# JuliaRobotics/KernelDensityEstimate.jl

Hardware: AMD Instinct MI355X
Metric: gibbs_product_samples_per_sec (higher is better)
Workload: dtype f64

## Files before the change

include/kdehip.h:

```cpp
#ifndef KDEHIP_H
#define KDEHIP_H

#include <stdint.h>

#ifdef __cplusplus
extern "C" {
#endif

#define KDEHIP_VERSION 600

enum {
  KDEHIP_OK = 0,
  KDEHIP_ERR_ARG = -1,
  KDEHIP_ERR_DIM_MISMATCH = -2,
  KDEHIP_ERR_RAND_SHORT = -3,
  KDEHIP_ERR_NO_DEVICE = -4,
  KDEHIP_ERR_HIP = -5,
  KDEHIP_ERR_ALLOC = -6,
  KDEHIP_ERR_UNSUPPORTED = -7
};

#define KDEHIP_MAX_DIMS 8
#define KDEHIP_MAX_DENS 16

// ... 19 lines not shown

int kdehip_gibbs1_trace(int Ndens, const kdehip_density *trees, int64_t Np, int Niter, double *pts,
                        int64_t *ind, const double *randU, int64_t nU, const double *randN, int64_t nN,
                        int addEntropy, int ndims, const uint8_t *partialDimMask, int device,
                        int32_t *labels);

int kdehip_gibbs1_multi(int Ndens, const kdehip_density *trees, int64_t Np, int Niter, double *pts,
                        int64_t *ind, const double *randU, int64_t nU, const double *randN, int64_t nN,
                        int addEntropy, int ndims, const uint8_t *partialDimMask, int device, int ngpus,
                        int32_t *labels);

#define KDEHIP_MANIFOLD_EUCLIDEAN 0
#define KDEHIP_MANIFOLD_CIRCULAR 1
int kdehip_gibbs1_manifold(int Ndens, const kdehip_density *trees, int64_t Np, int Niter, double *pts, int64_t *ind,
                           const double *randU, int64_t nU, const double *randN, int64_t nN, int addEntropy, int ndims,
                           const uint8_t *partialDimMask, const uint8_t *manifold , int device,
                           int32_t *labels );

int kdehip_prod_philox(int Ndens, const kdehip_density *trees, int64_t Np, int Niter, double *pts, int64_t *ind,
                       uint64_t seed, int addEntropy, int ndims, const uint8_t *partialDimMask, int precision,
                       int device, int ngpus, int32_t *labels);

typedef struct kdehip_product kdehip_product;

typedef struct kdehip_product_info_t {
  int32_t ndens, ndims, nlevels;
  int32_t precision;
  int64_t nodes_per_sweep;
  int64_t bytes_per_eval;
  int64_t packed_bytes;
  int32_t fast_math_path;
  int32_t device;
} kdehip_product_info_t;

int kdehip_product_create(kdehip_product **out, int Ndens, const kdehip_density *trees, int ndims,
                          const uint8_t *partialDimMask, int precision, int device);
void kdehip_product_destroy(kdehip_product *plan);
int kdehip_product_info(const kdehip_product *plan, kdehip_product_info_t *info);
int64_t kdehip_product_randu_per_sample(const kdehip_product *plan, int Niter);
int64_t kdehip_product_randn_per_sample(const kdehip_product *plan);

int kdehip_product_sample_streams(kdehip_product *plan, int64_t Np, int Niter,
                                  const double *d_randU, int64_t nU, const double *d_randN,
                                  int64_t nN, int addEntropy, double *d_points, int64_t *d_indices,
                                  int32_t *d_labels, void *stream);
int kdehip_product_sample_philox(kdehip_product *plan, int64_t Np, int Niter, uint64_t seed,
                                 int64_t sample_offset, int addEntropy, double *d_points,
                                 int64_t *d_indices, int32_t *d_labels, void *stream);
int kdehip_product_sample_philox_host(kdehip_product *plan, int64_t Np, int Niter, uint64_t seed,
                                      int64_t sample_offset, int addEntropy, double *points,
                                      int64_t *indices, int32_t *labels);
int64_t kdehip_product_fallback_count(kdehip_product *plan);
int kdehip_product_screen_stats(kdehip_product *plan, int32_t *levels, int64_t *steps, int64_t *repeats);
int kdehip_product_set_variant(kdehip_product *plan, int variant);
int kdehip_product_launch_geometry(const kdehip_product *plan, int64_t Np, int32_t *waves_per_workgroup,
                                   int32_t *waves_per_chain);
const char *kdehip_product_kernel_name(const kdehip_product *plan, int64_t Np);

typedef struct kdehip_product_multi kdehip_product_multi;
int kdehip_product_multi_create(kdehip_product_multi **out, int Ndens, const kdehip_density *trees, int ndims,
                                const uint8_t *partialDimMask, int precision, int first_device, int ngpus);
void kdehip_product_multi_destroy(kdehip_product_multi *mp);
int kdehip_product_multi_ngpus(const kdehip_product_multi *mp);
kdehip_product *kdehip_product_multi_plan(kdehip_product_multi *mp, int g);
int kdehip_product_multi_sample_philox(kdehip_product_multi *mp, int64_t Np, int Niter, uint64_t seed,
                                       int64_t sample_offset, int addEntropy, double *const *d_points,
                                       int64_t *const *d_indices, void *const *streams);
int kdehip_product_multi_transfers_per_product(const kdehip_product_multi *mp);

typedef struct kdehip_device_density kdehip_device_density;
int kdehip_density_upload(kdehip_device_density **out, const kdehip_density *host, int device);
void kdehip_density_free(kdehip_device_density *d);
int64_t kdehip_density_npts(const kdehip_device_density *d);
int kdehip_density_ndim(const kdehip_device_density *d);
int kdehip_prod_philox_device(int Ndens, kdehip_device_density *const *trees, int64_t Np, int Niter, uint64_t seed,
                              int64_t sample_offset, int addEntropy, const uint8_t *partialDimMask, int precision,
                              double *d_points, int64_t *d_indices, int32_t *d_labels, void *stream);

int kdehip_prod_philox_resident(int Ndens, kdehip_device_density *const *trees, int64_t Np, int Niter, uint64_t seed,
                                int addEntropy, const uint8_t *partialDimMask, int precision, double *pts, int64_t *ind);

int kdehip_density_from_device_points(kdehip_device_density **out, const double *d_points, int64_t D, int64_t N,
                                      int device, void *stream, double *bw_out, int32_t *nevals);
int kdehip_density_from_device_points_manifold(kdehip_device_density **out, const double *d_points, int64_t D, int64_t N,
                                               int device, void *stream, double *bw_out, int32_t *nevals,
                                               const uint8_t *manifold );
int kdehip_mul_device(kdehip_device_density **out, int Ndens, kdehip_device_density *const *trees, uint64_t seed,
                      int addEntropy, double *bw_out, int32_t *nevals);
typedef struct kdehip_mul_item {
  int32_t Ndens;
  int32_t addEntropy;
  kdehip_device_density *const *trees;
  uint64_t seed;
} kdehip_mul_item;
int kdehip_mul_device_batch(int nprod, const kdehip_mul_item *items, kdehip_device_density **out, double *bw_out,
                            int32_t *nevals);
int kdehip_density_download(const kdehip_device_density *d, double *centers, double *ranges, double *weights,
                            int64_t *left_child, int64_t *right_child, int64_t *lowest_leaf, int64_t *highest_leaf,
                            int64_t *permutation, double *means, double *bandwidth, double *bandwidthMin,
                            double *bandwidthMax, double *bw_out);

typedef struct kdehip_batch_item {
  int32_t Ndens;
  int32_t Niter;
  kdehip_device_density *const *trees;
  int64_t Np;
// ... 135 lines not shown
```

kerneldensityestimate.jl_amd/_lib.py:

```python
from __future__ import annotations

import ctypes as C
import os

_HERE = os.path.dirname(os.path.abspath(__file__))
LIB_PATH = os.environ.get("KDEHIP_LIB", os.path.join(_HERE, "libkdehip.so"))

f64p = C.POINTER(C.c_double)
i64p = C.POINTER(C.c_int64)
i32p = C.POINTER(C.c_int32)
u8p = C.POINTER(C.c_uint8)

KDEHIP_OK = 0
ERR_ARG, ERR_DIM_MISMATCH, ERR_RAND_SHORT, ERR_NO_DEVICE, ERR_HIP, ERR_ALLOC, ERR_UNSUPPORTED = -1, -2, -3, -4, -5, -6, -7
MAX_DIMS, MAX_DENS = 8, 16


class CDensity(C.Structure):
    _fields_ = [
        ("npts", C.c_int64), ("ndim", C.c_int64),
        ("means", f64p), ("bandwidth", f64p), ("weights", f64p),
        ("left_child", i64p), ("right_child", i64p), ("permutation", i64p),
    ]

# ... 25 lines not shown

class CSummaryItem(C.Structure):
    _fields_ = [("density", C.c_void_p), ("extend", C.c_double), ("Ngrid", C.c_int64), ("d_range", C.c_void_p),
                ("d_mean", C.c_void_p), ("d_cov", C.c_void_p), ("d_argmax", C.c_void_p), ("d_values", C.c_void_p)]


class CProductInfo(C.Structure):
    _fields_ = [
        ("ndens", C.c_int32), ("ndims", C.c_int32), ("nlevels", C.c_int32), ("precision", C.c_int32),
        ("nodes_per_sweep", C.c_int64), ("bytes_per_eval", C.c_int64), ("packed_bytes", C.c_int64),
        ("fast_math_path", C.c_int32), ("device", C.c_int32),
    ]


SIGNATURES = {
    "kdehip_version": (C.c_int, []),
    "kdehip_last_error": (C.c_char_p, []),
    "kdehip_device_count": (C.c_int, []),
    "kdehip_clear_cache": (None, []),
    "kdehip_gibbs1": (C.c_int, [C.c_int, C.POINTER(CDensity), C.c_int64, C.c_int, f64p, i64p, f64p, C.c_int64,
                                f64p, C.c_int64, C.c_int, C.c_int, u8p, C.c_int]),
    "kdehip_gibbs1_trace": (C.c_int, [C.c_int, C.POINTER(CDensity), C.c_int64, C.c_int, f64p, i64p, f64p, C.c_int64,
                                      f64p, C.c_int64, C.c_int, C.c_int, u8p, C.c_int, i32p]),
    "kdehip_gibbs1_multi": (C.c_int, [C.c_int, C.POINTER(CDensity), C.c_int64, C.c_int, f64p, i64p, f64p, C.c_int64,
                                      f64p, C.c_int64, C.c_int, C.c_int, u8p, C.c_int, C.c_int, i32p]),
    "kdehip_gibbs1_manifold": (C.c_int, [C.c_int, C.POINTER(CDensity), C.c_int64, C.c_int, f64p, i64p, f64p, C.c_int64,
                                         f64p, C.c_int64, C.c_int, C.c_int, u8p, u8p, C.c_int, i32p]),
    "kdehip_prod_philox": (C.c_int, [C.c_int, C.POINTER(CDensity), C.c_int64, C.c_int, f64p, i64p, C.c_uint64, C.c_int,
                                     C.c_int, u8p, C.c_int, C.c_int, C.c_int, i32p]),
    "kdehip_product_multi_create": (C.c_int, [C.POINTER(C.c_void_p), C.c_int, C.POINTER(CDensity), C.c_int, u8p,
                                              C.c_int, C.c_int, C.c_int]),
    "kdehip_product_multi_destroy": (None, [C.c_void_p]),
    "kdehip_product_multi_ngpus": (C.c_int, [C.c_void_p]),
    "kdehip_product_multi_plan": (C.c_void_p, [C.c_void_p, C.c_int]),
    "kdehip_product_multi_sample_philox": (C.c_int, [C.c_void_p, C.c_int64, C.c_int, C.c_uint64, C.c_int64, C.c_int,
                                                     C.POINTER(C.c_void_p), C.POINTER(C.c_void_p),
                                                     C.POINTER(C.c_void_p)]),
    "kdehip_product_multi_transfers_per_product": (C.c_int, [C.c_void_p]),
    "kdehip_product_create": (C.c_int, [C.POINTER(C.c_void_p), C.c_int, C.POINTER(CDensity), C.c_int, u8p,
                                        C.c_int, C.c_int]),
    "kdehip_product_destroy": (None, [C.c_void_p]),
    "kdehip_product_info": (C.c_int, [C.c_void_p, C.POINTER(CProductInfo)]),
    "kdehip_product_randu_per_sample": (C.c_int64, [C.c_void_p, C.c_int]),
    "kdehip_product_randn_per_sample": (C.c_int64, [C.c_void_p]),
    "kdehip_product_fallback_count": (C.c_int64, [C.c_void_p]),
    "kdehip_product_sample_streams": (C.c_int, [C.c_void_p, C.c_int64, C.c_int, C.c_void_p, C.c_int64,
                                                C.c_void_p, C.c_int64, C.c_int, C.c_void_p, C.c_void_p,
                                                C.c_void_p, C.c_void_p]),
    "kdehip_product_sample_philox": (C.c_int, [C.c_void_p, C.c_int64, C.c_int, C.c_uint64, C.c_int64, C.c_int,
                                               C.c_void_p, C.c_void_p, C.c_void_p, C.c_void_p]),
    "kdehip_product_sample_philox_host": (C.c_int, [C.c_void_p, C.c_int64, C.c_int, C.c_uint64, C.c_int64,
                                                    C.c_int, f64p, i64p, i32p]),
    "kdehip_product_screen_stats": (C.c_int, [C.c_void_p, i32p, i64p, i64p]),
    "kdehip_product_set_variant": (C.c_int, [C.c_void_p, C.c_int]),
    "kdehip_product_launch_geometry": (C.c_int, [C.c_void_p, C.c_int64, i32p, i32p]),
    "kdehip_product_kernel_name": (C.c_char_p, [C.c_void_p, C.c_int64]),
    "kdehip_density_upload": (C.c_int, [C.POINTER(C.c_void_p), C.POINTER(CDensity), C.c_int]),
    "kdehip_density_free": (None, [C.c_void_p]),
    "kdehip_density_npts": (C.c_int64, [C.c_void_p]),
    "kdehip_density_ndim": (C.c_int, [C.c_void_p]),
    "kdehip_prod_philox_device": (C.c_int, [C.c_int, C.POINTER(C.c_void_p), C.c_int64, C.c_int, C.c_uint64, C.c_int64,
                                            C.c_int, u8p, C.c_int, C.c_void_p, C.c_void_p, C.c_void_p, C.c_void_p]),
    "kdehip_prod_philox_resident": (C.c_int, [C.c_int, C.POINTER(C.c_void_p), C.c_int64, C.c_int, C.c_uint64, C.c_int, u8p,
                                              C.c_int, f64p, i64p]),
    "kdehip_philox_fill_uniform": (None, [C.c_uint64, C.c_int64, C.c_int64, C.c_int64, f64p]),
    "kdehip_philox_fill_normal": (None, [C.c_uint64, C.c_int64, C.c_int64, C.c_int64, f64p]),
    "kdehip_evaluate": (C.c_int, [C.POINTER(CDensity), f64p, C.c_int64, C.c_int, f64p, C.c_int]),
    "kdehip_eval_avg_logl": (C.c_int, [C.POINTER(CDensity), C.POINTER(CDensity), C.c_int, f64p, C.c_int]),
    "kdehip_eval_avg_logl_device_batch": (C.c_int, [C.c_int, C.POINTER(CLoglItem), C.c_void_p, C.c_void_p]),
    "kdehip_eval_avg_logl_device": (C.c_int, [C.c_void_p, C.c_void_p, C.c_int, f64p]),
    "kdehip_evaluate_device": (C.c_int, [C.c_void_p, C.c_void_p, C.c_int64, C.c_int, C.c_void_p, C.c_void_p]),
    "kdehip_evaluate_device_at": (C.c_int, [C.c_void_p, C.c_void_p, C.c_void_p, C.c_void_p]),
    "kdehip_evaluate_manifold": (C.c_int, [C.POINTER(CDensity), f64p, C.c_int64, C.c_int, f64p, C.c_int, u8p]),
    "kdehip_evaluate_device_manifold": (C.c_int, [C.c_void_p, C.c_void_p, C.c_int64, C.c_int, C.c_void_p, C.c_void_p, u8p]),
    "kdehip_evaluate_device_at_manifold": (C.c_int, [C.c_void_p, C.c_void_p, C.c_void_p, C.c_void_p, u8p]),
    "kdehip_eval_avg_logl_manifold": (C.c_int, [C.POINTER(CDensity), C.POINTER(CDensity), C.c_int, f64p, C.c_int, u8p]),
    "kdehip_eval_avg_logl_device_manifold": (C.c_int, [C.c_void_p, C.c_void_p, C.c_int, f64p, u8p]),
    "kdehip_eval_avg_logl_device_batch_manifold": (C.c_int, [C.c_int, C.POINTER(CLoglManifoldItem), C.c_void_p, C.c_void_p]),
    "kdehip_auto_bandwidth_manifold": (C.c_int, [C.c_int64, C.c_int64, f64p, f64p, i32p, C.c_int, u8p]),
    "kdehip_make_density_auto_manifold": (C.c_int, [C.c_int64, C.c_int64, f64p, f64p, i32p, C.c_int, f64p, f64p, f64p, i64p,
                                                    i64p, i64p, i64p, i64p, f64p, f64p, f64p, f64p, u8p]),
    "kdehip_density_from_device_points_manifold": (C.c_int, [C.POINTER(C.c_void_p), C.c_void_p, C.c_int64, C.c_int64,
                                                             C.c_int, C.c_void_p, f64p, i32p, u8p]),
    "kdehip_density_marginal_device": (C.c_int, [C.POINTER(C.c_void_p), C.c_void_p, C.c_int, i32p]),
    "kdehip_summary_device_batch": (C.c_int, [C.c_int, C.POINTER(CSummaryItem), C.c_void_p]),
    "kdehip_density_summary": (C.c_int, [C.c_void_p, f64p, C.c_int64, f64p, f64p, f64p, f64p, f64p]),
    "kdehip_kde_max": (C.c_int, [C.POINTER(CDensity), C.c_int64, f64p, f64p, C.c_int]),
    "kdehip_inters_intg_appx_is": (C.c_int, [C.POINTER(CDensity), C.POINTER(CDensity), C.c_int64, f64p, C.c_int]),
    "kdehip_inters_intg_appx_is_device": (C.c_int, [C.c_void_p, C.c_void_p, C.c_int64, f64p]),
    "kdehip_auto_bandwidth": (C.c_int, [C.c_int64, C.c_int64, f64p, f64p, i32p, C.c_int]),
    "kdehip_make_density_device_supported": (C.c_int, [C.c_int64, C.c_int64]),
    "kdehip_make_densities_device": (C.c_int, [C.c_int, C.c_int64, i64p] + [C.POINTER(C.c_void_p)] * 2 + [C.c_int64] +
                                     [C.POINTER(C.c_void_p)] * 13 + [C.c_int]),
    "kdehip_density_set_bandwidth": (C.c_int, [C.c_int64, C.c_int64, f64p, C.c_int64, f64p, i64p, i64p, f64p, f64p, f64p, f64p]),
    "kdehip_profile_sampler": (None, [C.c_int]),
    "kdehip_profile_phase_read": (C.c_int, [C.c_int, f64p, i64p]),
    "kdehip_selftest_fp32": (C.c_int, [C.c_int, C.c_uint32, C.c_uint64, C.c_int, f64p, C.POINTER(C.c_uint32),
                                      C.POINTER(C.c_uint32)]),
    "kdehip_profile_sampler_read": (C.c_int, [C.c_int, C.c_void_p, f64p, i64p]),
    "kdehip_product_multi_timing": (C.c_int, [C.c_void_p, f64p, f64p]),
    "kdehip_density_from_device_points": (C.c_int, [C.POINTER(C.c_void_p), C.c_void_p, C.c_int64, C.c_int64, C.c_int,
                                                    C.c_void_p, f64p, i32p]),
    "kdehip_mul_device": (C.c_int, [C.POINTER(C.c_void_p), C.c_int, C.POINTER(C.c_void_p), C.c_uint64, C.c_int, f64p, i32p]),
    "kdehip_mul_device_batch": (C.c_int, [C.c_int, C.POINTER(CMulItem), C.POINTER(C.c_void_p), f64p, i32p]),
    "kdehip_density_download": (C.c_int, [C.c_void_p, f64p, f64p, f64p, i64p, i64p, i64p, i64p, i64p, f64p, f64p, f64p,
                                          f64p, f64p]),
# ... 64 lines not shown
```

kerneldensityestimate.jl_amd/csrc/gibbs_lean.hip:

```cpp
#define KDEHIP_EXP256 1
#ifndef KDEHIP_PRELOAD_MAXB
#define KDEHIP_PRELOAD_MAXB 8
#endif
#include "gibbs_device.hpp"
#include "screen_device.hpp"

namespace kdehip {

template <int I> using IC = std::integral_constant<int, I>;
template <int N, int I = 0, typename F>
__device__ __forceinline__ void static_for(F &&f) {
  if constexpr (I < N) {
    f(IC<I>{});
    static_for<N, I + 1>(f);
  }
}

#if defined(KDEHIP_LEAN_HI) || (defined(KDEHIP_LEAN_DEV_M) && KDEHIP_LEAN_DEV_M > 4)
constexpr int kLeanMinDens = 8, kLeanMaxDens = 8;
#else
constexpr int kLeanMinDens = 2, kLeanMaxDens = 4;
#endif
constexpr int kLeanMaxNormals = 128;

__device__ __forceinline__ int scalar_copy(int x) {
  int y;
  asm("s_mov_b32 %0, %1" : "=s"(y) : "s"(x));
  return y;
}

template <int D>
struct LeanTile {
  int n;
  int flags;
  int lds_off;
  int stage_bytes;
  int chunk_rows;
  int seg;
  int hdr_lo, hdr_hi;
  int B, F, last_lane;
  int uniform_bw;
  __device__ __forceinline__ int64_t hdr_off() const {
    return (static_cast<int64_t>(hdr_hi) << 32) | static_cast<uint32_t>(hdr_lo);
  }
  __device__ __forceinline__ void load(const kdehip_v8i &d) {
    n = scalar_copy(d[0]);
    flags = scalar_copy(d[1]);
    lds_off = scalar_copy(d[2]);
    stage_bytes = scalar_copy(d[3]);
    chunk_rows = scalar_copy(d[4]);
    seg = scalar_copy(d[5]);
    hdr_lo = scalar_copy(d[6]);
    hdr_hi = scalar_copy(d[7]);
    B = (n + 63) >> 6;
    last_lane = flags & 0xFF;
    uniform_bw = flags >> 8;
    F = uniform_bw ? D + 1 : 2 * D + 1;
  }
};

template <typename P, typename T, bool OK> constexpr bool kCanPreloadImpl = OK && kIsLdsPtr<P> && sizeof(T) == 8;

template <typename T, int D, int M, int WAVES, bool BATCH = false, bool SCHUNK = false>
__global__ __launch_bounds__(WAVES * 64) void gibbs_lean_kernel(PlanDev plan_, RunArgs a_) {
  const LaunchView<BATCH> view(plan_, a_);
  const PlanDev &plan = view.plan;
  const auto &a = view.a;
  constexpr bool kPrefetchRows = (WAVES <= 12) || sizeof(T) == 4 || D <= 4;
  using RowPtr = std::conditional_t<(WAVES == 16 && sizeof(T) == 8), LdsPtrSplit<T>, LdsPtr<T>>;
  constexpr int kCopyWaves = WAVES > 4 ? 4 : WAVES;
  constexpr bool kKeptRows = (WAVES <= 8);
  constexpr bool kScreen = sizeof(T) == 8 && !BATCH;
  constexpr bool kPreloadBuild = kKeptRows && kPrefetchRows;
  constexpr int kNormOff = 2048;
  constexpr int kUnifOff = kNormOff + WAVES * kLeanMaxNormals * 8;
  constexpr int kPoolOff = kUnifOff + WAVES * 1024;
  constexpr bool kCoop = kScreen && SCHUNK && WAVES == 8;
  constexpr int kXchgOff = kPoolOff + kLdsPoolBytes;
  constexpr int kXchgSlotDoubles = 32 + 4 * 64;
  constexpr int kXchgBytes = kCoop ? 64 + WAVES * kXchgSlotDoubles * 8 : 0;
  static_assert(kPoolOff + kLdsPoolBytes + kXchgBytes <= 160 * 1024, "LDS budget of one CU exceeded");
  __shared__ __attribute__((aligned(1024))) unsigned char smem[kPoolOff + kLdsPoolBytes + kXchgBytes];

  double *sExpTab = reinterpret_cast<double *>(smem);
  if (threadIdx.x < 256) sExpTab[threadIdx.x] = kExp2Tab256[threadIdx.x];
  if constexpr (kCoop) {
    if (threadIdx.x < 16) reinterpret_cast<int *>(smem + kXchgOff)[threadIdx.x] = 0;
  }

  const int lane = threadIdx.x & 63;
  const int wave = __builtin_amdgcn_readfirstlane(static_cast<int>(threadIdx.x >> 6));
  KDEHIP_PRIO_CHAIN();
  const int chain = wave;
  int64_t s = static_cast<int64_t>(view.block) * WAVES + chain;
  const bool live = s < a.Np;
  if (!live) s = a.Np - 1;
  const uint64_t gs = static_cast<uint64_t>(a.sample_offset + s);
  const void *fb = live ? static_cast<const void *>(plan.levels) : nullptr;

  const int L = plan.L;
  const T *__restrict__ data = static_cast<const T *>(plan.data);
  const LevelTable levels{(const __attribute__((address_space(4))) kdehip_v16i *)(plan.levels)};
  const StepTable steps{(const __attribute__((address_space(4))) kdehip_v8i *)(plan.levels + 2 * plan.M * (plan.L + 1))};
  unsigned char *pool = smem + kPoolOff;
  const int dl = lane < D ? lane : D - 1;
  const int vlev = a.variant % 1000;

  double *sNorm = reinterpret_cast<double *>(smem + kNormOff) + chain * kLeanMaxNormals;
  const int R = D * (L + 1);
  if (a.rng_philox) {
    for (int b = lane; 2 * b < R; b += 64) {
      double n0, n1;
// ... 636 lines not shown
      const int nsteps = npass * M;
      for (int p = 0; p < npass; ++p)
        static_for<M>([&](auto jc) {
          constexpr int j = decltype(jc)::value;
          constexpr int jn = (j + 1 == M) ? 0 : j + 1;
          const LeanTile<D> ds = tile(j);
          const LeanTile<D> dn = tile(jn);
          T mean = x, cov = T(0);
          if (p != 0) product(jc, mean, cov);
          const double u = next_uniform();
          const T *hdr = data + ds.hdr_off();
          const int pos = draw(ds, hdr, mean, cov, [&](const auto &ev) {
            using Ev = std::decay_t<decltype(ev)>;
            const int RS = TileAddr<T>::stride(ds.F), rc = ds.chunk_rows;
            LaneAcc<T> acc;
            SegSums<T> seg;
            const int cps = seg_chunks(ds.seg);
            const bool use_seg = cps != 0;
            int cin = 0;
            KDEHIP_PRIO_ROWS();
            for (int r0 = 0; r0 < ds.B; r0 += rc, ++gchunk) {
              staging_barrier();
              if (r0 + rc < ds.B) stage_chunk(ds, r0 + rc, (gchunk + 1) & 1);
              else if (t + 1 < nsteps) stage_chunk(dn, 0, (gchunk + 1) & 1);
              const int nrows = (ds.B - r0 < rc) ? (ds.B - r0) : rc;
              const auto crows = (RowPtr)(pool + (gchunk & 1) * (kLdsPoolBytes / 2));
              lane_rows_all<T, RowPtr, Ev, kPrefetchRows>(crows, nrows, RS, lane, ev, acc);
              if (use_seg && ++cin == cps) { seg.note(acc.total()); cin = 0; }
            }
            KDEHIP_PRIO_CHAIN();
            const T S = acc.total();
            if (use_seg)
              return __builtin_amdgcn_readfirstlane(
                  select_or_raise_seg<T, const T *>(S, seg, cps * rc, hdr + kTileHeader, ds, lane, ev, u, fb));
            return __builtin_amdgcn_readfirstlane(select_or_raise<T, const T *>(S, hdr + kTileHeader, ds, lane, ev, u, fb));
          });
          adopt(jc, ds, hdr, pos);
          ++t;
        });
    } else {
      for (int p = 0; p < npass; ++p)
        static_for<M>([&](auto jc) {
          const LeanTile<D> ds = tile(decltype(jc)::value);
          step(jc, ds, data + ds.hdr_off(), p == 0, x);
        });
    }

    if (tabulated) {
      TabDesc td[M];
      static_for<M>([&](auto jc) { td[decltype(jc)::value] = tabs[decltype(jc)::value * (L + 1) + l]; });
      uint32_t word = 0;
      static_for<M>([&](auto jc) { word |= static_cast<uint32_t>(psel[decltype(jc)::value]) << td[decltype(jc)::value].shift; });
      word = __builtin_amdgcn_readfirstlane(word);
      for (int p = 1; p <= a.Niter; ++p)
        static_for<M>([&](auto jc) {
          constexpr int j = decltype(jc)::value;
          const TabDesc &tj = td[j];
          const uint32_t cfg = (word & ((1u << tj.shift) - 1u)) | ((word >> (tj.shift + tj.bits)) << tj.shift);
          const T *row = tables + tj.off + static_cast<int64_t>(cfg) * (tj.n + 1);
          const int n = tj.n;
          const T incl = row[lane < n ? lane : n];
          const double u = next_uniform();
          const T total = lane_read(incl, n < 64 ? n : 63);
          int pos;
          if (!(total >= Num<T>::tiny_total())) {
            count_fallback(fb, lane);
            const LeanTile<D> dk = tile(j);
            const T wl = ((LdsPtr<T>)(pool + dk.lds_off) + kTileHeader)[(dk.F - 1) * TileAddr<T>::kField + (n - 1) * TileAddr<T>::kLane];
            int z = n - 1;
            if (wl > T(0)) {
              z = static_cast<int>(ceil(u * static_cast<double>(n))) - 1;
              z = z < 0 ? 0 : (z > n - 1 ? n - 1 : z);
            }
            pos = __builtin_amdgcn_readfirstlane(z);
          } else {
            const T target = static_cast<T>(u) * total;
            unsigned long long hit = __ballot(target <= incl);
            if (n < 64) hit &= (1ull << n) - 1ull;
            pos = hit ? (__ffsll(hit) - 1) : (n - 1);
          }
          word = (word & ~(((1u << tj.bits) - 1u) << tj.shift)) | (static_cast<uint32_t>(pos) << tj.shift);
        });
      static_for<M>([&](auto jc) {
        constexpr int j = decltype(jc)::value;
        const int pk = static_cast<int>((word >> td[j].shift) & ((1u << td[j].bits) - 1u));
        const LeanTile<D> dk = tile(j);
        adopt(jc, dk, (LdsPtr<T>)(pool + dk.lds_off), pk);
      });
    }
    if (a.labels && live && lane == 0) {
      static_for<M>([&](auto jc) {
        constexpr int j = decltype(jc)::value;
        a.labels[(s * M + j) * L + (l - 1)] = plan.perm[levels[j * (L + 1) + l].perm_off + psel[j]];
      });
    }
    if (l == L && live && lane == 0) {
      static_for<M>([&](auto jc) {
        constexpr int j = decltype(jc)::value;
        const int64_t label = static_cast<int64_t>(plan.perm[levels[j * (L + 1) + l].perm_off + psel[j]]) + 1;
        a.indices[s * M + j] = label;
        for (int k = 0; k < a.npeers; ++k) a.peer_indices[k][s * M + j] = label;
      });
    }
  }

#ifdef KDEHIP_SCREEN_STAMPS
  if (view.block == 3 && wave == 5 && lane == 0)
    for (int k = 0; k < 8; ++k) { g_screen_stamps[k] = sstamp[k]; g_screen_stamps[8 + k] = rstamp[k]; }
#endif
  if constexpr (kScreen) {
    if (live && lane == 0 && n_screened != 0u) {
      unsigned long long *cnt = reinterpret_cast<unsigned long long *>(const_cast<LevelDesc *>(plan.levels));
      atomicAdd(cnt - 3, static_cast<unsigned long long>(n_screened));
      if (n_repeated != 0u) atomicAdd(cnt - 2, static_cast<unsigned long long>(n_repeated));
    }
  }
  {
    T mean, cov;
    product(IC<-1>{}, mean, cov);
    T xf = mean;
    if (a.addEntropy) xf = mean + Num<T>::sqrt(cov) * static_cast<T>(sNorm[L * D + dl]);
    if (live && lane < D) {
      a.points[s * D + lane] = static_cast<double>(xf);
      for (int k = 0; k < a.npeers; ++k) a.peer_points[k][s * D + lane] = static_cast<double>(xf);
    }
  }
}


template <typename T, int D, int M, int WAVES>
static void launch_lean_waves(const PlanDev &plan, const RunArgs &args, hipStream_t stream) {
  const int64_t blocks = (args.Np + WAVES - 1) / WAVES;
  if constexpr (sizeof(T) == 8 && WAVES >= 8) {
    if (M == 8 || (plan.screened == 2 && args.use_screen)) {
      hipLaunchKernelGGL((gibbs_lean_kernel<T, D, M, WAVES, false, true>), dim3(static_cast<unsigned>(blocks)), dim3(WAVES * 64),
// ... 135 lines not shown
```

kerneldensityestimate.jl_amd/csrc/kdehip_internal.hpp:

```cpp
#pragma once

#include <hip/hip_runtime_api.h>

#include <cstddef>
#include <cstdint>
#include <functional>
#include <string>
#include <vector>

#include "../../include/kdehip.h"

namespace kdehip {

int set_error(int code, const std::string &msg);
const char *last_error_cstr();

constexpr int kTileHeader = 8;
#if defined(__HIPCC__)
#define KDEHIP_TILE_HD __host__ __device__ inline
#else
#define KDEHIP_TILE_HD inline
#endif
template <int ELEM_BYTES>
struct TileAddrBytes {
// ... 15 lines not shown
  kStageStream = 2,
  kStageChunked = 3,
  kStageScreen = 4,
  kStageScreenStream = 5,
  kStageScreenChunked = 6
};
constexpr int kLdsPoolBytes = 120 * 1024;

struct LevelDesc {
  int32_t n;
  int32_t B;
  int32_t F;
  int32_t uniform_bw;
  int64_t hdr_off;
  int64_t perm_off;
  uint32_t mask_bits;
  uint32_t others_bits;
  int32_t stage_mode;
  int32_t lds_off;
  int32_t stage_bytes;
  int32_t last_lane;
  int32_t chunk_rows;
  int32_t seg;
};
constexpr int kMaxSegDesc = 8;
inline int32_t seg_geometry(int B, int rc) {
  if (rc <= 0 || rc > 64) return 0;
  const int cps = 64 / rc, sr = cps * rc, nseg = (B + sr - 1) / sr;
  return nseg <= kMaxSegDesc ? (cps | (nseg << 16)) : 0;
}
static_assert(sizeof(LevelDesc) == 64, "LevelDesc is read with scalar loads; keep it 64 bytes");

struct StepDesc {
  int32_t n;
  int32_t flags;
  int32_t lds_off;
  int32_t stage_bytes;
  int32_t chunk_rows;
  int32_t seg;
  int32_t hdr_lo, hdr_hi;
};
static_assert(sizeof(StepDesc) == 32, "StepDesc is read with one 32-byte scalar load");

constexpr int kScreenHeaderFloats = 48;
constexpr int kScreenMaxRows = 64;
constexpr int kScreenMaxRowsChunked = 128;
constexpr float kScreenMaxAbsMean = 65536.0f;
constexpr double kScreenMinVar = 1.0 / 128.0, kScreenMaxVar = 256.0;
constexpr float kScreenMaxNa = 0x1p-11f;
constexpr float kScreenMaxA2 = 1.14e7f;

struct TabDesc {
  int64_t off;
  int64_t row_base;
  int32_t n;
  int32_t ncfg;
  int32_t shift;
  int32_t bits;
};
static_assert(sizeof(TabDesc) == 32, "TabDesc is read with one 32-byte scalar load");
constexpr int64_t kTabMaxEntries = 512 * 1024;
constexpr int64_t kTabMinChains = 16;

struct PlanDev {
  const void *data;
  const int32_t *perm;
  const LevelDesc *levels;
  const void *tables;
  const TabDesc *tabdesc;
  int64_t tab_rows_total;
  int32_t M, L, D, Lt;
  int32_t screened;
  uint32_t circ_bits;
  int32_t reserved_[2];
};

constexpr int kMaxPeers = 7;
struct BatchEntry;
struct RunArgs {
  int64_t Np;
  int32_t Niter;
  int32_t addEntropy;
  int32_t rng_philox;
  int32_t variant;
  int32_t table_build;
  int32_t use_tables;
  int32_t use_screen;
  const double *randU;
  const double *randN;
  int64_t K, R;
  int64_t nU, nN;
  uint64_t seed;
  int64_t sample_offset;
  double *points;
  int64_t *indices;
  int32_t *labels;
  int32_t npeers;
  double *peer_points[kMaxPeers];
  int64_t *peer_indices[kMaxPeers];
  const BatchEntry *batch;
  const int32_t *batch_map;
};

struct BatchPlanHead {
  const void *data;
  const int32_t *perm;
  const LevelDesc *levels;
  const void *tables;
  const TabDesc *tabdesc;
  int64_t tab_rows_total;
  int32_t M, L, D, Lt;
};
struct BatchRun {
// ... 98 lines not shown
```

kerneldensityestimate.jl_amd/csrc/pack_levels.cpp:

```cpp
#include <cmath>
#include <cstdlib>
#include <cstring>

#include "device_density.hpp"
#include "host_pool.hpp"
#include "kdehip_internal.hpp"

namespace kdehip {

namespace {
thread_local std::string g_err;
}

int set_error(int code, const std::string &msg) {
  g_err = msg;
  return code;
}
const char *last_error_cstr() { return g_err.c_str(); }

int nlevels_for(int64_t maxNp) {
  return static_cast<int>(std::floor(std::log(static_cast<double>(maxNp)) / std::log(2.0) + 1.0));
}

bool variances_in_range(const double *bw_lo, const double *bw_hi, int D, int precision) {
// ... 289 lines not shown
        const int64_t bytes = ((kScreenHeaderFloats + TileAddrBytes<4>::body(ds.B, ds.F)) * 4 + 1023) / 1024 * 1024;
        sum += bytes;
        mx = bytes > mx ? bytes : mx;
      }
      static const bool stream_on = [] { const char *e = std::getenv("KDEHIP_SCREEN_STREAM"); return !(e && e[0] == '0'); }();
      static const bool chunk_on = [] { const char *e = std::getenv("KDEHIP_SCREEN_CHUNK"); return !(e && e[0] == '0'); }();
      const bool together = sum <= kLdsPoolBytes && maxB <= kScreenMaxRows;
      const bool streamed = !together && stream_on && mx <= kLdsPoolBytes / 2 && maxB <= kScreenMaxRows;
      const bool chunked = !together && !streamed && stream_on && chunk_on;
      if (!ok || !(together || streamed || chunked)) continue;
      int64_t off = 0;
      for (int j = 0; j < M; ++j) {
        const LevelDesc &ds = out.levels[static_cast<size_t>(j) * (L + 1) + l];
        LevelDesc &sc = scr[static_cast<size_t>(j) * (L + 1) + l];
        sc.n = ds.n; sc.B = ds.B; sc.F = ds.F; sc.uniform_bw = ds.uniform_bw; sc.last_lane = ds.last_lane;
        sc.stage_mode = together ? kStageScreen : streamed ? kStageScreenStream : kStageScreenChunked;
        if (chunked) {
          const int64_t pair_bytes = TileAddrBytes<4>::stride(ds.F) * 4;
          const int64_t cp = ((kLdsPoolBytes / 2 - kScreenHeaderFloats * 4) / pair_bytes) & ~int64_t(1);
          sc.chunk_rows = static_cast<int32_t>(2 * cp);
        }
        felem = (felem + 63) & ~int64_t(63);
        sc.hdr_off = felem;
        const int64_t elems = kScreenHeaderFloats + TileAddrBytes<4>::body(ds.B, ds.F);
        felem += elems;
        sc.stage_bytes = static_cast<int32_t>((elems * 4 + 1023) / 1024 * 1024);
        sc.lds_off = together ? static_cast<int32_t>(off) : 0;
        off += sc.stage_bytes;
      }
      ++out.nscreened;
    }
    if (out.nscreened > 0) {
      out.screens.swap(scr);
      nelem = (felem + 1) / 2;
    }
  }
  out.data_elems = nelem + 1024 / 4;
  out.steps.resize(out.levels.size());
  for (size_t idx = 0; idx < out.levels.size(); ++idx) {
    const LevelDesc &ds = out.levels[idx];
    StepDesc &s = out.steps[idx];
    s.n = ds.n;
    s.flags = ds.last_lane | (ds.uniform_bw << 8);
    s.lds_off = ds.lds_off;
    if (!out.screens.empty() && out.screens[idx].stage_mode == kStageScreen) s.lds_off = out.screens[idx].lds_off;
    s.stage_bytes = ds.stage_bytes;
    s.chunk_rows = ds.chunk_rows;
    s.seg = ds.seg;
    s.hdr_lo = static_cast<int32_t>(ds.hdr_off & 0xFFFFFFFF);
    s.hdr_hi = static_cast<int32_t>(ds.hdr_off >> 32);
  }

  out.tabdesc.assign(static_cast<size_t>(M) * (L + 1), TabDesc{});
  for (auto &t : out.tabdesc) t.off = -1;
  if (out.fast && M >= 2) {
    int64_t entries = 0, rows = 0;
    for (int l = 1; l <= L; ++l) {
      bool ok = true;
      int total_bits = 0;
      std::vector<int> bits(M, 0);
      for (int j = 0; j < M && ok; ++j) {
        const LevelDesc &dj = out.levels[static_cast<size_t>(j) * (L + 1) + l];
        if (dj.B != 1 || dj.stage_mode != kStageResident || (dj.n & (dj.n - 1)) != 0) { ok = false; break; }
        while ((1 << bits[j]) < dj.n) ++bits[j];
        total_bits += bits[j];
      }
      if (!ok || total_bits > 30) break;
      int64_t lvl_entries = 0;
      for (int j = 0; j < M; ++j)
        lvl_entries += (int64_t(1) << (total_bits - bits[j])) * ((int64_t(1) << bits[j]) + 1);
      if (entries + lvl_entries > kTabMaxEntries) break;
      int shift = 0;
      for (int j = 0; j < M; ++j) {
        TabDesc &td = out.tabdesc[static_cast<size_t>(j) * (L + 1) + l];
        td.n = 1 << bits[j];
        td.bits = bits[j];
        td.shift = shift;
        shift += bits[j];
        td.ncfg = 1 << (total_bits - bits[j]);
        td.off = entries;
        td.row_base = rows;
        entries += static_cast<int64_t>(td.ncfg) * (td.n + 1);
        rows += td.ncfg;
      }
      out.Lt = l;
    }
    out.tab_entries = entries;
    out.tab_rows = rows;
  }
  return KDEHIP_OK;
}


struct FillFindings {
  bool bad = false;
  double lo[KDEHIP_MAX_DIMS], hi[KDEHIP_MAX_DIMS];
  FillFindings() { for (int d = 0; d < KDEHIP_MAX_DIMS; ++d) { lo[d] = INFINITY; hi[d] = 0.0; } }
};

template <typename T>
static void fill_density(const PackedProduct &pp, const kdehip_density &t, int j, int l0, int l1, T *data, int32_t *perm,
                         FillFindings &f) {
  const int D = pp.D, L = pp.L;
  bool bad = false;
  double *lo = f.lo, *hi = f.hi;
  for (int l = l0; l < l1; ++l) {
    const size_t idx = static_cast<size_t>(j) * (L + 1) + l;
    const LevelDesc &ds = pp.levels[idx];
    const int32_t *cur = pp.front.data() + pp.front_off[idx];
    const int64_t n = ds.n, B = ds.B;
    const int F = ds.F;
    const bool uni = ds.uniform_bw != 0;
    using TA = TileAddr<T>;
    const int64_t RS = TA::stride(F);
    T *hdr = data + ds.hdr_off;
    for (int d = 0; d < kTileHeader; ++d)
      hdr[d] = d < D ? static_cast<T>(t.bandwidth[(static_cast<int64_t>(cur[0]) - 1) * D + d]) : T(0);
    for (int d = 0; d < D; ++d) {
      const double v = t.bandwidth[(static_cast<int64_t>(cur[0]) - 1) * D + d];
      bad |= !(v > 0.0) | !(v < INFINITY);
      lo[d] = v < lo[d] ? v : lo[d];
      hi[d] = v > hi[d] ? v : hi[d];
    }
    T *tile = hdr + kTileHeader;
    int32_t *prow = perm + ds.perm_off;
    for (int64_t i = 0; i < B; ++i) {
      int64_t src[64];
      for (int ln = 0; ln < 64; ++ln) {
        const int64_t z = static_cast<int64_t>(ln) * B + i;
        src[ln] = z < n ? static_cast<int64_t>(cur[z]) - 1 : -1;
      }
      T *row = tile + TA::row(i, RS);
      T dst[64];
      auto put = [&](int f) {
        for (int ln = 0; ln < 64; ++ln) row[f * TA::kField + ln * TA::kLane] = dst[ln];
// ... 108 lines not shown
```

kerneldensityestimate.jl_amd/csrc/product.hip:

```cpp
#include <hip/hip_runtime.h>

#include <atomic>
#include <cstdlib>
#include <chrono>
#include <cstdio>
#include <cstdlib>
#include <cstring>
#include <deque>
#include <mutex>
#include <new>
#include <string>
#include <vector>

#include "device_density.hpp"
#include "entry_helpers.hpp"
#include "kdehip_internal.hpp"
#include "phase_timer.hpp"

namespace kdehip { extern std::atomic<unsigned> g_peer_epoch; }
#include "philox.hpp"

using namespace kdehip;

struct kdehip_product {
// ... 338 lines not shown
    if (plan->d_work) cached_free(plan->d_work, plan->work_cap);
  }
  delete plan;
}

int kdehip_product_info(const kdehip_product *plan, kdehip_product_info_t *info) {
  if (!plan || !info) return set_error(KDEHIP_ERR_ARG, "null argument");
  info->ndens = plan->host.M;
  info->ndims = plan->host.D;
  info->nlevels = plan->host.L;
  info->precision = plan->precision;
  info->nodes_per_sweep = plan->host.nodes_per_sweep;
  info->bytes_per_eval = (2 * plan->host.D + 1) * (plan->precision == 64 ? 8 : 4);
  info->packed_bytes = plan->packed_bytes;
  info->fast_math_path = plan->fast ? 1 : 0;
  info->device = plan->device;
  return KDEHIP_OK;
}

int64_t kdehip_product_randu_per_sample(const kdehip_product *plan, int Niter) {
  if (!plan || Niter < 0) return -1;
  return static_cast<int64_t>(plan->host.M) * (1 + static_cast<int64_t>(plan->host.L) * (Niter + 1));
}
int64_t kdehip_product_randn_per_sample(const kdehip_product *plan) {
  if (!plan) return -1;
  return static_cast<int64_t>(plan->host.D) * (plan->host.L + 1);
}

int64_t kdehip_product_fallback_count(kdehip_product *plan) {
  if (!plan) return set_error(KDEHIP_ERR_ARG, "null plan");
  DeviceGuard guard;
  int rc = guard.enter(plan->device);
  if (rc != KDEHIP_OK) return rc;
  unsigned long long v = 0;
  KDEHIP_CHECK(hipDeviceSynchronize());
  KDEHIP_CHECK(hipMemcpy(&v, plan->d_fallbacks, sizeof(v), hipMemcpyDeviceToHost));
  return static_cast<int64_t>(v);
}

int kdehip_product_screen_stats(kdehip_product *plan, int32_t *levels, int64_t *steps, int64_t *repeats) {
  if (!plan) return set_error(KDEHIP_ERR_ARG, "null plan");
  DeviceGuard guard;
  const int rc = guard.enter(plan->device);
  if (rc != KDEHIP_OK) return rc;
  unsigned long long v[2] = {0, 0};
  KDEHIP_CHECK(hipDeviceSynchronize());
  KDEHIP_CHECK(hipMemcpy(v, plan->d_fallbacks - 2, sizeof(v), hipMemcpyDeviceToHost));
  if (levels) *levels = plan->dev.screened ? plan->host.nscreened : 0;
  if (steps) *steps = static_cast<int64_t>(v[0]);
  if (repeats) *repeats = static_cast<int64_t>(v[1]);
  return KDEHIP_OK;
}

int kdehip_product_set_variant(kdehip_product *plan, int variant) {
  if (!plan) return set_error(KDEHIP_ERR_ARG, "null plan");
  plan->variant = variant;
  return KDEHIP_OK;
}

int kdehip_product_launch_geometry(const kdehip_product *plan, int64_t Np, int32_t *waves_per_workgroup,
                                   int32_t *waves_per_chain) {
  if (!plan || !waves_per_workgroup || !waves_per_chain) return set_error(KDEHIP_ERR_ARG, "null argument");
  DeviceGuard guard;
  const int rc = guard.enter(plan->device);
  if (rc != KDEHIP_OK) return rc;
  const bool lean = plan->mode == kModeFast && ((plan->host.M >= 2 && plan->host.M <= 4) || (plan->host.M == 8 && plan->precision == 64));
  const int v = plan->variant % 1000;
  const bool as_lean = lean && !(v >= kVariantGenericBase && v < kVariantGenericBase + 20);
  *waves_per_workgroup = as_lean ? lean_waves(Np, plan->variant) : chains_per_workgroup(Np, plan->variant);
  *waves_per_chain = 1;
  return KDEHIP_OK;
}

const char *kdehip_product_kernel_name(const kdehip_product *plan, int64_t Np) {
  if (!plan) return "";
  const int v = plan->variant % 1000;
  const bool forced_general = (v >= kVariantGenericBase && v < kVariantGenericBase + 20);
  const int M = plan->host.M, L = plan->host.L, D = plan->host.D;
  bool lean = !forced_general && plan->mode == kModeFast && D * (L + 1) <= 128 &&
              ((M >= 2 && M <= 4) || (M == 8 && plan->precision == 64));
  if (lean && M == 8) {
    DeviceGuard guard;
    if (guard.enter(plan->device) != KDEHIP_OK) return "";
    lean = lean_waves(Np, plan->variant) != 4;
  }
  return lean ? "gibbs_lean_kernel" : "gibbs_product_kernel";
}

int kdehip_product_sample_streams(kdehip_product *plan, int64_t Np, int Niter, const double *d_randU,
                                  int64_t nU, const double *d_randN, int64_t nN, int addEntropy,
                                  double *d_points, int64_t *d_indices, int32_t *d_labels,
                                  void *stream) {
  const int rc = enqueue_streams(plan, Np, Niter, d_randU, nU, d_randN, nN, addEntropy, d_points, d_indices,
                                 d_labels, stream);
  if (rc == KDEHIP_OK && Np > 0) plan->async_pending.store(true);
  return rc;
}

int kdehip_product_sample_philox(kdehip_product *plan, int64_t Np, int Niter, uint64_t seed,
                                 int64_t sample_offset, int addEntropy, double *d_points,
                                 int64_t *d_indices, int32_t *d_labels, void *stream) {
  const int rc = enqueue_philox(plan, Np, Niter, seed, sample_offset, addEntropy, d_points, d_indices, d_labels,
                                stream);
  if (rc == KDEHIP_OK && Np > 0) plan->async_pending.store(true);
  return rc;
}
// ... 971 lines not shown
```

kerneldensityestimate.jl_amd/product.py:

```python
from __future__ import annotations

import ctypes as C
import math
import os

import numpy as np

from . import _lib
from ._lib import f64p, i64p, i32p, u8p, ptr
from .density import BallTreeDensity, Ndim, Npts


def _mask_array(partialDimMask, Ndens, ndims):
    if partialDimMask is None:
        return None
    m = np.ascontiguousarray(np.asarray(partialDimMask, dtype=bool).reshape(Ndens, ndims).astype(np.uint8))
    return m


def nlevels(maxNp: int) -> int:
    return int(math.floor(math.log(float(maxNp)) / math.log(2.0) + 1.0))


class ProductPlan:
# ... 6 lines not shown
        arr = (_lib.CDensity * self.Ndens)(*[t._cstruct() for t in trees])
        mask = _mask_array(partialDimMask, self.Ndens, self.ndims)
        h = C.c_void_p()
        _lib.check(_lib.lib.kdehip_product_create(C.byref(h), self.Ndens, arr, self.ndims,
                                                  None if mask is None else ptr(mask, u8p),
                                                  int(precision), int(device)))
        self._h = h
        info = _lib.CProductInfo()
        _lib.check(_lib.lib.kdehip_product_info(self._h, C.byref(info)))
        self.nlevels = info.nlevels
        self.precision = info.precision
        self.nodes_per_sweep = info.nodes_per_sweep
        self.bytes_per_eval = info.bytes_per_eval
        self.packed_bytes = info.packed_bytes
        self.fast_math_path = bool(info.fast_math_path)
        self.device = info.device

    def close(self):
        if getattr(self, "_h", None):
            _lib.lib.kdehip_product_destroy(self._h)
            self._h = None

    def __del__(self):
        try:
            self.close()
        except Exception:
            pass

    def __enter__(self):
        return self

    def __exit__(self, *exc):
        self.close()

    def randu_per_sample(self, Niter: int) -> int:
        return int(_lib.lib.kdehip_product_randu_per_sample(self._h, int(Niter)))

    def randn_per_sample(self) -> int:
        return int(_lib.lib.kdehip_product_randn_per_sample(self._h))

    def evals_per_sample(self, Niter: int) -> int:
        return (int(Niter) + 1) * int(self.nodes_per_sweep)

    def fallback_count(self) -> int:
        n = int(_lib.lib.kdehip_product_fallback_count(self._h))
        if n < 0:
            _lib.check(n)
        return n

    def screen_stats(self) -> dict:
        lv, st, rp = C.c_int32(0), C.c_int64(0), C.c_int64(0)
        _lib.check(_lib.lib.kdehip_product_screen_stats(self._h, C.byref(lv), C.byref(st), C.byref(rp)))
        return {"levels": int(lv.value), "steps": int(st.value), "repeats": int(rp.value)}

    def set_variant(self, v: int):
        _lib.check(_lib.lib.kdehip_product_set_variant(self._h, int(v)))

    def kernel_name(self, Np: int) -> str:
        return _lib.lib.kdehip_product_kernel_name(self._h, int(Np)).decode()

    def launch_geometry(self, Np: int) -> dict:
        w, t = C.c_int32(0), C.c_int32(0)
        _lib.check(_lib.lib.kdehip_product_launch_geometry(self._h, int(Np), C.byref(w), C.byref(t)))
        return {"waves": int(w.value), "team": int(t.value)}

    @staticmethod
    def _addr(x):
        if x is None:
            return None
        if hasattr(x, "data_ptr"):
            return C.c_void_p(x.data_ptr())
        return C.c_void_p(int(x))

    def sample_philox_device(self, Np, Niter, seed, sample_offset, addEntropy, d_points, d_indices,
                             d_labels=None, stream=None):
        _lib.check(_lib.lib.kdehip_product_sample_philox(
            self._h, int(Np), int(Niter), C.c_uint64(int(seed) & (2 ** 64 - 1)), int(sample_offset),
            int(bool(addEntropy)), self._addr(d_points), self._addr(d_indices), self._addr(d_labels),
            self._addr(stream)))

    def sample_streams_device(self, Np, Niter, d_randU, nU, d_randN, nN, addEntropy, d_points, d_indices,
                              d_labels=None, stream=None):
        _lib.check(_lib.lib.kdehip_product_sample_streams(
            self._h, int(Np), int(Niter), self._addr(d_randU), int(nU), self._addr(d_randN), int(nN),
            int(bool(addEntropy)), self._addr(d_points), self._addr(d_indices), self._addr(d_labels),
            self._addr(stream)))

    def sample(self, Np, Niter=3, seed=0, sample_offset=0, addEntropy=True, want_labels=False):
        D, M, L = self.ndims, self.Ndens, self.nlevels
        pts = np.zeros(D * Np)
        ind = np.ones(M * Np, dtype=np.int64)
        labels = np.zeros(Np * M * L, dtype=np.int32) if want_labels else None
        _lib.check(_lib.lib.kdehip_product_sample_philox_host(
            self._h, int(Np), int(Niter), C.c_uint64(int(seed) & (2 ** 64 - 1)), int(sample_offset),
            int(bool(addEntropy)), ptr(pts, f64p), ptr(ind, i64p),
            None if labels is None else ptr(labels, i32p)))
        out = (pts.reshape(Np, D).T.copy(), ind.reshape(Np, M).T.copy())
        if want_labels:
            out = out + (labels.reshape(Np, M, L),)
        return out


class MultiProductPlan:

    def __init__(self, trees, partialDimMask=None, precision=64, first_device=0, ngpus=1, ndims=None):
        trees = list(trees)
# ... 417 lines not shown
```

Measured before the change: 4.274 million.

## Stage Gibbs cumulative-weight tables into LDS via buffer-load-to-LDS

```diff
diff --git a/include/kdehip.h b/include/kdehip.h
--- a/include/kdehip.h
+++ b/include/kdehip.h
@@ -95,6 +95,7 @@
                                       int64_t *indices, int32_t *labels);
 int64_t kdehip_product_fallback_count(kdehip_product *plan);
 int kdehip_product_screen_stats(kdehip_product *plan, int32_t *levels, int64_t *steps, int64_t *repeats);
+int kdehip_product_table_placement(const kdehip_product *plan, int32_t *levels, int32_t *lds_off);
 int kdehip_product_set_variant(kdehip_product *plan, int variant);
 int kdehip_product_launch_geometry(const kdehip_product *plan, int64_t Np, int32_t *waves_per_workgroup,
                                    int32_t *waves_per_chain);
diff --git a/kerneldensityestimate.jl_amd/_lib.py b/kerneldensityestimate.jl_amd/_lib.py
--- a/kerneldensityestimate.jl_amd/_lib.py
+++ b/kerneldensityestimate.jl_amd/_lib.py
@@ -101,6 +101,7 @@
     "kdehip_product_sample_philox_host": (C.c_int, [C.c_void_p, C.c_int64, C.c_int, C.c_uint64, C.c_int64,
                                                     C.c_int, f64p, i64p, i32p]),
     "kdehip_product_screen_stats": (C.c_int, [C.c_void_p, i32p, i64p, i64p]),
+    "kdehip_product_table_placement": (C.c_int, [C.c_void_p, i32p, i32p]),
     "kdehip_product_set_variant": (C.c_int, [C.c_void_p, C.c_int]),
     "kdehip_product_launch_geometry": (C.c_int, [C.c_void_p, C.c_int64, i32p, i32p]),
     "kdehip_product_kernel_name": (C.c_char_p, [C.c_void_p, C.c_int64]),
diff --git a/kerneldensityestimate.jl_amd/csrc/gibbs_lean.hip b/kerneldensityestimate.jl_amd/csrc/gibbs_lean.hip
--- a/kerneldensityestimate.jl_amd/csrc/gibbs_lean.hip
+++ b/kerneldensityestimate.jl_amd/csrc/gibbs_lean.hip
@@ -58,6 +58,18 @@
     F = uniform_bw ? D + 1 : 2 * D + 1;
   }
 };
+
+template <int WAVES>
+__device__ __forceinline__ void stage_table(const unsigned char *__restrict__ src, unsigned char *dst, int valid, int wave,
+                                            int lane) {
+  const __amdgpu_buffer_rsrc_t rsrc =
+      __builtin_amdgcn_make_buffer_rsrc(const_cast<unsigned char *>(src), 0, valid, 0x00020000);
+  const int pieces = (valid + 1023) >> 10;
+  for (int c = wave; c < pieces; c += WAVES) {
+    const int off = __builtin_amdgcn_readfirstlane(c << 10);
+    __builtin_amdgcn_raw_ptr_buffer_load_lds(rsrc, (LdsVoidPtr)(dst + off), 16, lane << 4, off, 0, 0);
+  }
+}
 
 template <typename P, typename T, bool OK> constexpr bool kCanPreloadImpl = OK && kIsLdsPtr<P> && sizeof(T) == 8;
 
@@ -800,35 +812,66 @@
       uint32_t word = 0;
       static_for<M>([&](auto jc) { word |= static_cast<uint32_t>(psel[decltype(jc)::value]) << td[decltype(jc)::value].shift; });
       word = __builtin_amdgcn_readfirstlane(word);
-      for (int p = 1; p <= a.Niter; ++p)
-        static_for<M>([&](auto jc) {
-          constexpr int j = decltype(jc)::value;
-          const TabDesc &tj = td[j];
-          const uint32_t cfg = (word & ((1u << tj.shift) - 1u)) | ((word >> (tj.shift + tj.bits)) << tj.shift);
-          const T *row = tables + tj.off + static_cast<int64_t>(cfg) * (tj.n + 1);
-          const int n = tj.n;
-          const T incl = row[lane < n ? lane : n];
-          const double u = next_uniform();
-          const T total = lane_read(incl, n < 64 ? n : 63);
-          int pos;
-          if (!(total >= Num<T>::tiny_total())) {
-            count_fallback(fb, lane);
-            const LeanTile<D> dk = tile(j);
-            const T wl = ((LdsPtr<T>)(pool + dk.lds_off) + kTileHeader)[(dk.F - 1) * TileAddr<T>::kField + (n - 1) * TileAddr<T>::kLane];
-            int z = n - 1;
-            if (wl > T(0)) {
-              z = static_cast<int>(ceil(u * static_cast<double>(n))) - 1;
-              z = z < 0 ? 0 : (z > n - 1 ? n - 1 : z);
+      constexpr bool kTabLds = M <= kTabLdsMaxDens;
+      int nlds = 0;
+      if constexpr (kTabLds) {
+        static_for<M>([&](auto jc) { nlds += td[decltype(jc)::value].lds_off >= 0 ? 1 : 0; });
+        if (nlds != 0) {
+          static_for<M>([&](auto jc) {
+            const TabDesc &tj = td[decltype(jc)::value];
+            if (tj.lds_off >= 0) {
+              const int lead = tab_lds_lead(tj.off, int(sizeof(T)));
+              stage_table<WAVES>(reinterpret_cast<const unsigned char *>(tables + tj.off) - lead, pool + tj.lds_off - lead,
+                                 lead + tj.ncfg * (tj.n + 1) * int(sizeof(T)), wave, lane);
             }
-            pos = __builtin_amdgcn_readfirstlane(z);
-          } else {
-            const T target = static_cast<T>(u) * total;
-            unsigned long long hit = __ballot(target <= incl);
-            if (n < 64) hit &= (1ull << n) - 1ull;
-            pos = hit ? (__ffsll(hit) - 1) : (n - 1);
+          });
+          staging_barrier();
+        }
+      }
+      auto tab_step = [&](auto jc, auto base) {
+        constexpr int j = decltype(jc)::value;
+        const TabDesc &tj = td[j];
+        const uint32_t cfg = (word & ((1u << tj.shift) - 1u)) | ((word >> (tj.shift + tj.bits)) << tj.shift);
+        const auto row = base + static_cast<std::conditional_t<kIsLdsPtr<decltype(base)>, int, int64_t>>(cfg) * (tj.n + 1);
+        const int n = tj.n;
+        const T incl = row[lane < n ? lane : n];
+        const double u = next_uniform();
+        const T total = lane_read(incl, n < 64 ? n : 63);
+        int pos;
+        if (!(total >= Num<T>::tiny_total())) {
+          count_fallback(fb, lane);
+          const LeanTile<D> dk = tile(j);
+          const T wl = ((LdsPtr<T>)(pool + dk.lds_off) + kTileHeader)[(dk.F - 1) * TileAddr<T>::kField + (n - 1) * TileAddr<T>::kLane];
+          int z = n - 1;
+          if (wl > T(0)) {
+            z = static_cast<int>(ceil(u * static_cast<double>(n))) - 1;
+            z = z < 0 ? 0 : (z > n - 1 ? n - 1 : z);
           }
-          word = (word & ~(((1u << tj.bits) - 1u) << tj.shift)) | (static_cast<uint32_t>(pos) << tj.shift);
+          pos = __builtin_amdgcn_readfirstlane(z);
+        } else {
+          const T target = static_cast<T>(u) * total;
+          unsigned long long hit = __ballot(target <= incl);
+          if (n < 64) hit &= (1ull << n) - 1ull;
+          pos = hit ? (__ffsll(hit) - 1) : (n - 1);
+        }
+        word = (word & ~(((1u << tj.bits) - 1u) << tj.shift)) | (static_cast<uint32_t>(pos) << tj.shift);
+      };
+      auto sweeps = [&](auto kc) {
+        constexpr int K = decltype(kc)::value;
+        for (int p = 1; p <= a.Niter; ++p)
+          static_for<M>([&](auto jc) {
+            constexpr int j = decltype(jc)::value;
+            if constexpr (j < K) tab_step(jc, (LdsPtr<T>)(pool + td[j].lds_off));
+            else tab_step(jc, tables + td[j].off);
+          });
+      };
+      if constexpr (kTabLds) {
+        static_for<M + 1>([&](auto kc) {
+          if (nlds == decltype(kc)::value) sweeps(kc);
         });
+      } else {
+        sweeps(IC<0>{});
+      }
       static_for<M>([&](auto jc) {
         constexpr int j = decltype(jc)::value;
         const int pk = static_cast<int>((word >> td[j].shift) & ((1u << td[j].bits) - 1u));
diff --git a/kerneldensityestimate.jl_amd/csrc/kdehip_internal.hpp b/kerneldensityestimate.jl_amd/csrc/kdehip_internal.hpp
--- a/kerneldensityestimate.jl_amd/csrc/kdehip_internal.hpp
+++ b/kerneldensityestimate.jl_amd/csrc/kdehip_internal.hpp
@@ -91,13 +91,19 @@
 
 struct TabDesc {
   int64_t off;
-  int64_t row_base;
+  int32_t row_base;
+  int32_t lds_off;
   int32_t n;
   int32_t ncfg;
   int32_t shift;
   int32_t bits;
 };
 static_assert(sizeof(TabDesc) == 32, "TabDesc is read with one 32-byte scalar load");
+constexpr int kTabLdsMaxDens = 4;
+KDEHIP_TILE_HD constexpr int tab_lds_lead(int64_t off, int esz) { return static_cast<int>((off * esz) & 15); }
+KDEHIP_TILE_HD constexpr int64_t tab_lds_span(int64_t off, int64_t entries, int esz) {
+  return (tab_lds_lead(off, esz) + entries * esz + 1023) & ~int64_t(1023);
+}
 constexpr int64_t kTabMaxEntries = 512 * 1024;
 constexpr int64_t kTabMinChains = 16;
 
diff --git a/kerneldensityestimate.jl_amd/csrc/pack_levels.cpp b/kerneldensityestimate.jl_amd/csrc/pack_levels.cpp
--- a/kerneldensityestimate.jl_amd/csrc/pack_levels.cpp
+++ b/kerneldensityestimate.jl_amd/csrc/pack_levels.cpp
@@ -365,7 +365,7 @@
   }
 
   out.tabdesc.assign(static_cast<size_t>(M) * (L + 1), TabDesc{});
-  for (auto &t : out.tabdesc) t.off = -1;
+  for (auto &t : out.tabdesc) { t.off = -1; t.lds_off = -1; }
   if (out.fast && M >= 2) {
     int64_t entries = 0, rows = 0;
     for (int l = 1; l <= L; ++l) {
@@ -384,6 +384,13 @@
         lvl_entries += (int64_t(1) << (total_bits - bits[j])) * ((int64_t(1) << bits[j]) + 1);
       if (entries + lvl_entries > kTabMaxEntries) break;
       int shift = 0;
+      int64_t lds_end = 0;
+      for (int j = 0; j < M; ++j) lds_end += out.levels[static_cast<size_t>(j) * (L + 1) + l].stage_bytes;
+#ifdef KDEHIP_X_NO_TABLES_LDS
+      bool place = false;
+#else
+      bool place = M <= kTabLdsMaxDens && out.all_active;
+#endif
       for (int j = 0; j < M; ++j) {
         TabDesc &td = out.tabdesc[static_cast<size_t>(j) * (L + 1) + l];
         td.n = 1 << bits[j];
@@ -392,8 +399,15 @@
         shift += bits[j];
         td.ncfg = 1 << (total_bits - bits[j]);
         td.off = entries;
-        td.row_base = rows;
-        entries += static_cast<int64_t>(td.ncfg) * (td.n + 1);
+        td.row_base = static_cast<int32_t>(rows);
+        const int64_t tab_entries = static_cast<int64_t>(td.ncfg) * (td.n + 1);
+        const int64_t span = tab_lds_span(td.off, tab_entries, static_cast<int>(esz));
+        place = place && lds_end + span <= kLdsPoolBytes;
+        if (place) {
+          td.lds_off = static_cast<int32_t>(lds_end) + tab_lds_lead(td.off, static_cast<int>(esz));
+          lds_end += span;
+        }
+        entries += tab_entries;
         rows += td.ncfg;
       }
       out.Lt = l;
diff --git a/kerneldensityestimate.jl_amd/csrc/product.hip b/kerneldensityestimate.jl_amd/csrc/product.hip
--- a/kerneldensityestimate.jl_amd/csrc/product.hip
+++ b/kerneldensityestimate.jl_amd/csrc/product.hip
@@ -414,6 +414,17 @@
   return KDEHIP_OK;
 }
 
+int kdehip_product_table_placement(const kdehip_product *plan, int32_t *levels, int32_t *lds_off) {
+  if (!plan) return set_error(KDEHIP_ERR_ARG, "null plan");
+  const int M = plan->host.M, L = plan->host.L, Lt = plan->dev.Lt;
+  if (levels) *levels = Lt;
+  if (lds_off)
+    for (int j = 0; j < M; ++j)
+      for (int l = 1; l <= L; ++l)
+        lds_off[j * L + (l - 1)] = (l <= Lt) ? plan->host.tabdesc[static_cast<size_t>(j) * (L + 1) + l].lds_off : -1;
+  return KDEHIP_OK;
+}
+
 int kdehip_product_set_variant(kdehip_product *plan, int variant) {
   if (!plan) return set_error(KDEHIP_ERR_ARG, "null plan");
   plan->variant = variant;
diff --git a/kerneldensityestimate.jl_amd/product.py b/kerneldensityestimate.jl_amd/product.py
--- a/kerneldensityestimate.jl_amd/product.py
+++ b/kerneldensityestimate.jl_amd/product.py
@@ -82,6 +82,12 @@
         lv, st, rp = C.c_int32(0), C.c_int64(0), C.c_int64(0)
         _lib.check(_lib.lib.kdehip_product_screen_stats(self._h, C.byref(lv), C.byref(st), C.byref(rp)))
         return {"levels": int(lv.value), "steps": int(st.value), "repeats": int(rp.value)}
+
+    def table_placement(self) -> dict:
+        lv = C.c_int32(0)
+        off = np.full(self.Ndens * self.nlevels, -1, dtype=np.int32)
+        _lib.check(_lib.lib.kdehip_product_table_placement(self._h, C.byref(lv), ptr(off, i32p)))
+        return {"levels": int(lv.value), "lds_off": off.reshape(self.Ndens, self.nlevels)}
 
     def set_variant(self, v: int):
         _lib.check(_lib.lib.kdehip_product_set_variant(self._h, int(v)))
```

New measurement: 4.210 million. 0.985x the previous value.
